# TIGER-AI-Lab/AnyV2V

Measured on NVIDIA H100. Metric: denoising-steps/sec (16f x 512^2 I2VGen-XL, 50 inv + 50 edit PnP sampling), higher is better.
Workload: dtype f16

## Files before the change

anyv2v_b200/csrc/gemm_common.cuh:

```cuda
#pragma once
#include "host_util.cuh"
#include "ptx.cuh"

namespace av2v {

struct GemmP {
  int mode;
  const __half* a;
  const __half* a2;
  const __half* w;
  int M, N, K;
  int lda, lda2, k_split;
  int Hin, Win, chan;
  int Ho, Wo, stride;
  int taps_w, up2, py, px;
  int Cin;
  int F, HW;
  const __half* bias;
  const __half* rowbias;
  int rows_per_rowbias;
  const __half* residual;
  __half* out;
  int ldo;
  int n_slots;
  long long slot_stride;
  int geglu;
  int n_tiles, num_kb;
};

__device__ __forceinline__ float gelu_erf_fast(float g) {
  const float z = fabsf(g) * 0.70710678118654752f;
  float t;
  asm("rcp.approx.ftz.f32 %0, %1;" : "=f"(t) : "f"(fmaf(0.5f, z, 1.0f)));
  float p = fmaf(t, 0.22427836f, -0.69402432f);
  p = fmaf(p, t, 0.45475456f);
  p = fmaf(p, t, 0.26681793f);
  p = fmaf(p, t, 1.01429605f);
  p = fmaf(p, t, -1.26611602f);
  const float e = t * ex2_approx(fmaf(-z, z, p) * 1.4426950408889634f);
  return fmaf(-fabsf(0.5f * g), e, fmaxf(g, 0.0f));
}

__device__ __forceinline__ uint32_t stage_offset(int row, int chunk) {
  return static_cast<uint32_t>(row * 256 + ((chunk ^ (row & 7)) << 4));
}


template <bool kConv>
__device__ __forceinline__ long long out_row_offset(const GemmP& p, int m) {
  if (!kConv || !p.up2) return static_cast<long long>(m) * p.ldo;
  const int j = m % p.Wo, t = m / p.Wo, i = t % p.Ho, n = t / p.Ho;
  return ((static_cast<long long>(n) * 2 * p.Ho + 2 * i + p.py) * (2 * p.Wo) + 2 * j + p.px) * p.ldo;
}

template <bool kConv>
__device__ __forceinline__ void fetch_residual_band(const GemmP& p, int slot, int m0, int n0, int r0, uint32_t tile) {
  const int lane = threadIdx.x & 31, ch = lane & 15;
  const int c = n0 + 8 * ch;
  const __half* src = p.residual + slot * p.slot_stride + c;
#pragma unroll
  for (int i = 0; i < 8; ++i) {
    const int r = r0 + 2 * i + (lane >> 4);
    const bool v = m0 + r < p.M && c < p.N;
    cp_async16(tile + stage_offset(r, ch), v ? src + out_row_offset<kConv>(p, m0 + r) : p.residual, v);
  }
}

template <int kBands>
__device__ __forceinline__ void epilogue_bands(const GemmP& p, const float (&d)[kBands][64], int m0, int n0, int r0,
                                               uint32_t tile) {
  const int fr = r0 + ((threadIdx.x & 31) >> 2);
  const int cq = 2 * (threadIdx.x & 3);
  const __half* rb[kBands][2];
#pragma unroll
  for (int b = 0; b < kBands; ++b)
#pragma unroll
    for (int h = 0; h < 2; ++h) {
      const int m = m0 + fr + 64 * b + 8 * h;
      rb[b][h] = p.rowbias && m < p.M ? p.rowbias + static_cast<long long>(m / p.rows_per_rowbias) * p.N : nullptr;
    }
#pragma unroll
  for (int j = 0; j < 16; ++j) {
    const int c = n0 + 8 * j + cq;
    if (c >= p.N) continue;
    float2 bias = make_float2(0.f, 0.f);
    if (p.bias) bias = __half22float2(*reinterpret_cast<const __half2*>(p.bias + c));
#pragma unroll
    for (int b = 0; b < kBands; ++b)
#pragma unroll
      for (int h = 0; h < 2; ++h) {
        const uint32_t at = tile + stage_offset(fr + 64 * b + 8 * h, j) + 2 * cq;
        float o0 = d[b][4 * j + 2 * h], o1 = d[b][4 * j + 2 * h + 1];
        if (p.bias) {
          o0 += bias.x;
          o1 += bias.y;
        }
        if (rb[b][h]) {
          const float2 t = __half22float2(*reinterpret_cast<const __half2*>(rb[b][h] + c));
          o0 += t.x;
          o1 += t.y;
        }
        if (p.residual) {
          const uint32_t rr = ld_shared_u32(at);
          const float2 r = __half22float2(*reinterpret_cast<const __half2*>(&rr));
          o0 += r.x;
          o1 += r.y;
        }
        st_shared_u32(at, pack_half2(o0, o1));
      }
  }
}

template <bool kConv>
__device__ __forceinline__ void copy_out_band(const GemmP& p, int slot, int m0, int n0, int r0, uint32_t tile) {
  const int lane = threadIdx.x & 31;
  const bool geglu = !kConv && p.geglu;
  const int lg = geglu ? 3 : 4;
  const int col0 = geglu ? n0 / 2 : n0, n_out = geglu ? p.N / 2 : p.N;
  __half* out = p.out + slot * p.slot_stride + col0;
#pragma unroll
  for (int i = 0; i < 8; ++i) {
    const int idx = 32 * i + lane;
    const int r = r0 + (idx >> lg), ch = idx & ((1 << lg) - 1);
    if ((idx >> lg) < 16 && m0 + r < p.M && col0 + 8 * ch < n_out)
      st_global_v4(out + out_row_offset<kConv>(p, m0 + r) + 8 * ch, ld_shared_v4(tile + stage_offset(r, ch)));
  }
}

int gemm_linear_ws(const GemmP& p, int tiles, cudaStream_t stream);
bool conv_ws_box(const GemmP& p, unsigned (&box)[3]);
int gemm_conv_ws(const GemmP& p, const unsigned (&box)[3], int tiles, cudaStream_t stream);

}
```

anyv2v_b200/csrc/gemm_wgmma.cu:

```cuda
#include "gemm_common.cuh"

namespace av2v {
namespace {

constexpr int BM = 128, BN = 128, BK = 64;
constexpr int kStages = 3;
constexpr int kThreads = 256;
constexpr int kTileBytes = BM * BK * 2;
constexpr int kSmemBytes = kStages * 2 * kTileBytes + 1024;

struct ARows {
  long long base[4];
  int y[4], x[4];
};

__device__ __forceinline__ void a_rows_init(const GemmP& p, int m0, int r0, ARows& ar) {
#pragma unroll
  for (int i = 0; i < 4; ++i) {
    const int m = m0 + r0 + 32 * i;
    ar.y[i] = -1 << 20;
    ar.x[i] = 0;
    ar.base[i] = 0;
    if (m >= p.M) continue;
    if (p.mode == AV2V_A_CONV3X3) {
      const int ox = m % p.Wo, t = m / p.Wo, oy = t % p.Ho, n = t / p.Ho;
      const int y0 = p.up2 ? oy - 1 + p.py : oy * p.stride - 1;
      const int x0 = p.up2 ? ox - 1 + p.px : ox * p.stride - 1;
      ar.y[i] = y0;
      ar.x[i] = x0;
      ar.base[i] = (static_cast<long long>(n) * p.Hin + y0) * p.Win + x0;
    } else {
      ar.base[i] = m;
      ar.y[i] = (m % (p.F * p.HW)) / p.HW;
    }
  }
}

__device__ __forceinline__ void load_stage(const GemmP& p, const ARows& ar, int kb, int n0, uint32_t sA, uint32_t sB) {
  const int tid = threadIdx.x;
  const int ch = tid & 7, r0 = tid >> 3;
  const int k0 = kb * BK;
  if (p.mode == AV2V_A_CONV3X3) {
    const int tap = k0 / p.Cin, c = k0 - tap * p.Cin + ch * 8;
    const int ky = tap / p.taps_w, kx = tap - ky * p.taps_w;
    const bool cval = c < p.chan;
#pragma unroll
    for (int i = 0; i < 4; ++i) {
      const int y = ar.y[i] + ky, x = ar.x[i] + kx;
      const bool v = cval && y >= 0 && y < p.Hin && x >= 0 && x < p.Win;
      const __half* src = p.a + (ar.base[i] + static_cast<long long>(ky) * p.Win + kx) * p.chan + c;
      cp_async16(sA + sw128_offset(r0 + 32 * i, ch), v ? src : p.a, v);
    }
  } else {
    const int kt = k0 / p.Cin, c = k0 - kt * p.Cin + ch * 8;
#pragma unroll
    for (int i = 0; i < 4; ++i) {
      const int f = ar.y[i] + kt - 1;
      const bool v = ar.y[i] >= 0 && f >= 0 && f < p.F;
      const __half* src = p.a + (ar.base[i] + static_cast<long long>(kt - 1) * p.HW) * p.Cin + c;
      cp_async16(sA + sw128_offset(r0 + 32 * i, ch), v ? src : p.a, v);
    }
  }
  const bool kval = k0 + ch * 8 < p.K;
#pragma unroll
  for (int i = 0; i < 4; ++i) {
    const int n = n0 + r0 + 32 * i;
    const bool v = kval && n < p.N;
    cp_async16(sB + sw128_offset(r0 + 32 * i, ch), v ? p.w + static_cast<long long>(n) * p.K + k0 + ch * 8 : p.w, v);
  }
}

__global__ void __launch_bounds__(kThreads, 2) gemm_wgmma_kernel(const __grid_constant__ GemmP p) {
  extern __shared__ uint8_t smem_raw[];
  uint8_t* smem = reinterpret_cast<uint8_t*>((reinterpret_cast<uintptr_t>(smem_raw) + 1023) & ~uintptr_t(1023));
  const uint32_t s0 = smem_u32(smem);
  auto sA = [&](int s) { return s0 + static_cast<uint32_t>(s) * 2 * kTileBytes; };
  auto sB = [&](int s) { return s0 + static_cast<uint32_t>(s) * 2 * kTileBytes + kTileBytes; };

  const int n_t = blockIdx.x % p.n_tiles;
  const int m_t = blockIdx.x / p.n_tiles;
  const int m0 = m_t * BM, n0 = n_t * BN;
  const int wg = threadIdx.x >> 7;

  ARows ar;
  a_rows_init(p, m0, threadIdx.x >> 3, ar);

  float d[1][64];
#pragma unroll
  for (int i = 0; i < 64; ++i) d[0][i] = 0.f;

  const int nk = p.num_kb;
#pragma unroll
  for (int s = 0; s < kStages - 2; ++s) {
    if (s < nk) load_stage(p, ar, s, n0, sA(s), sB(s));
    cp_async_commit();
  }
  for (int kb = 0; kb < nk; ++kb) {
    cp_async_wait<kStages - 3>();
    fence_proxy_async_smem();
    __syncthreads();
    {
      const int pf = kb + kStages - 2;
      if (pf < nk) load_stage(p, ar, pf, n0, sA(pf % kStages), sB(pf % kStages));
      cp_async_commit();
    }
    const int s = kb % kStages;
    const uint32_t a_base = sA(s) + wg * 64 * 128;
    const uint32_t b_base = sB(s);
    wgmma_fence();
#pragma unroll
    for (int k = 0; k < BK / 16; ++k)
      wgmma_m64n128_ss(d[0], sw128_desc(a_base + k * 32), sw128_desc(b_base + k * 32), 1);
    wgmma_commit();
    wgmma_wait<1>();
    reg_fence(d[0]);
  }
  const int r0 = 16 * (threadIdx.x >> 5);
  if (p.residual) fetch_residual_band<true>(p, 0, m0, n0, r0, sA(nk % kStages));
  wgmma_wait<0>();
  reg_fence(d[0]);

  const int n_res = p.residual ? p.n_slots : 1;
  if (n_res > 1) {
    __syncthreads();
    for (int s = 1; s < n_res; ++s) fetch_residual_band<true>(p, s, m0, n0, r0, sA((nk + s) % kStages));
  }
  cp_async_commit();
  cp_async_wait<0>();
  __syncwarp();
  for (int s = 0; s < n_res; ++s) epilogue_bands<1>(p, d, m0, n0, r0, sA((nk + s) % kStages));
  __syncwarp();
  for (int s = 0; s < p.n_slots; ++s) copy_out_band<true>(p, s, m0, n0, r0, sA((nk + (p.residual ? s : 0)) % kStages));
}

}
}

using namespace av2v;

extern "C" int av2v_gemm_f16(const av2v_gemm_args* a, av2v_stream_t stream_) {
  cudaStream_t stream = static_cast<cudaStream_t>(stream_);
  AV2V_REQUIRE(a != nullptr, AV2V_EINVAL, "gemm: null args");
  AV2V_REQUIRE(a->a && a->w && a->out, AV2V_EINVAL, "gemm: null a/w/out pointer");
  AV2V_REQUIRE(a->M > 0 && a->N > 0 && a->K > 0, AV2V_EINVAL, "gemm: M,N,K must be positive (%d,%d,%d)", a->M, a->N,
               a->K);
  AV2V_REQUIRE(a->N % 8 == 0 && a->K % 8 == 0, AV2V_EINVAL, "gemm: N and K must be multiples of 8 (%d,%d)", a->N,
               a->K);
  AV2V_REQUIRE((a->geglu || a->ldo >= a->N) && a->ldo % 8 == 0, AV2V_EINVAL,
               "gemm: ldo must be >= N and a multiple of 8");
  AV2V_REQUIRE(a->n_slots >= 1, AV2V_EINVAL, "gemm: n_slots must be >= 1");
  AV2V_REQUIRE(!a->residual || a->n_slots <= kStages, AV2V_ENOSUP, "gemm: at most %d slots with a residual (one staging tile each)", kStages);
  AV2V_REQUIRE(a->n_slots == 1 || a->slot_stride % 8 == 0, AV2V_EALIGN, "gemm: slot_stride must be a multiple of 8");
  AV2V_REQUIRE(aligned16(a->a) && aligned16(a->w) && aligned16(a->out), AV2V_EALIGN,
               "gemm: a/w/out must be 16-byte aligned");
  AV2V_REQUIRE(!a->bias || aligned16(a->bias), AV2V_EALIGN, "gemm: bias must be 16-byte aligned");
  AV2V_REQUIRE(!a->rowbias || (aligned16(a->rowbias) && a->rows_per_rowbias > 0), AV2V_EALIGN,
               "gemm: rowbias must be 16-byte aligned with rows_per_rowbias > 0");
  AV2V_REQUIRE(!a->residual || aligned16(a->residual), AV2V_EALIGN, "gemm: residual must be 16-byte aligned");

  GemmP p{};
  p.mode = a->mode;
  p.a = static_cast<const __half*>(a->a);
  p.w = static_cast<const __half*>(a->w);
  p.M = a->M;
  p.N = a->N;
  p.K = a->K;
  p.bias = static_cast<const __half*>(a->bias);
  p.rowbias = static_cast<const __half*>(a->rowbias);
  p.rows_per_rowbias = a->rows_per_rowbias;
  p.residual = static_cast<const __half*>(a->residual);
  p.out = static_cast<__half*>(a->out);
  p.ldo = a->ldo;
  p.n_slots = a->n_slots;
  p.slot_stride = a->slot_stride;
  p.geglu = a->geglu ? 1 : 0;
  p.stride = 1;
  p.taps_w = 3;
  if (a->geglu) {
    AV2V_REQUIRE(a->mode == AV2V_A_LINEAR, AV2V_EINVAL, "gemm/geglu: LINEAR mode only");
    AV2V_REQUIRE(a->N % 64 == 0, AV2V_EINVAL, "gemm/geglu: N must be a multiple of 64 (got %d)", a->N);
    AV2V_REQUIRE(!a->residual && !a->rowbias && a->n_slots == 1, AV2V_EINVAL, "gemm/geglu: no residual / rowbias / slots");
    AV2V_REQUIRE(a->ldo >= a->N / 2, AV2V_EINVAL, "gemm/geglu: ldo must be >= N/2");
  }
  if (a->mode == AV2V_A_LINEAR) {
    AV2V_REQUIRE((a->a2 != nullptr || a->lda >= a->K) && a->lda % 8 == 0, AV2V_EINVAL, "gemm: lda must be >= K and a multiple of 8");
    p.lda = a->lda;
    p.k_split = a->K;
    if (a->a2 != nullptr) {
      AV2V_REQUIRE(a->k_split > 0 && a->k_split < a->K && a->k_split % BK == 0, AV2V_EINVAL,
                   "gemm: k_split must be a multiple of 64 inside (0, K) (got %d, K = %d)", a->k_split, a->K);
      AV2V_REQUIRE(a->lda >= a->k_split && a->lda2 >= a->K - a->k_split && a->lda2 % 8 == 0 && aligned16(a->a2), AV2V_EINVAL,
                   "gemm: a / a2 row strides must cover their column ranges (multiples of 8), a2 16-byte aligned");
      p.a2 = static_cast<const __half*>(a->a2);
      p.lda2 = a->lda2;
      p.k_split = a->k_split;
    }
    AV2V_REQUIRE(a->n_slots == 1, AV2V_ENOSUP, "gemm/linear: one output slot only (got n_slots = %d)", a->n_slots);
  } else if (a->mode == AV2V_A_CONV3X3) {
    AV2V_REQUIRE(a->NF > 0 && a->H > 0 && a->W > 0 && a->Cin > 0, AV2V_EINVAL, "gemm/conv3x3: bad geometry");
    AV2V_REQUIRE(a->Cin % BK == 0, AV2V_ENOSUP, "gemm/conv3x3: Cin must be a multiple of 64 (got %d)", a->Cin);
    const int up = a->up2_phase;
    AV2V_REQUIRE(up >= 0 && up <= 4, AV2V_EINVAL, "gemm/conv3x3: up2_phase must be 0..4 (got %d)", up);
    AV2V_REQUIRE(a->K == (up ? 4 : 9) * a->Cin, AV2V_EINVAL, "gemm/conv3x3: K must equal 9*Cin (4*Cin for an up2 phase)");
    AV2V_REQUIRE(!up || (a->stride <= 1 && !a->rowbias && !a->residual && a->n_slots == 1), AV2V_EINVAL,
                 "gemm/conv3x3: an up2 phase takes bias only (no stride, rowbias, residual, slots)");
    const int stride = a->stride == 0 ? 1 : a->stride;
    AV2V_REQUIRE(stride == 1 || stride == 2, AV2V_ENOSUP, "gemm/conv3x3: stride must be 1 or 2 (got %d)", a->stride);
    AV2V_REQUIRE(a->H % stride == 0 && a->W % stride == 0, AV2V_ENOSUP, "gemm/conv3x3: H, W must be multiples of the stride");
    const int chan = a->a_channels == 0 ? a->Cin : a->a_channels;
    AV2V_REQUIRE(chan > 0 && chan <= a->Cin && chan % 8 == 0, AV2V_EINVAL, "gemm/conv3x3: a_channels must be a multiple of 8 in (0, Cin]");
    AV2V_REQUIRE(static_cast<long long>(a->NF) * (a->H / stride) * (a->W / stride) == a->M, AV2V_EINVAL,
                 "gemm/conv3x3: M != NF*(H/stride)*(W/stride)");
    p.Hin = a->H;
    p.Win = a->W;
    p.chan = chan;
    p.Ho = a->H / stride;
    p.Wo = a->W / stride;
    p.stride = stride;
    p.Cin = a->Cin;
    if (up) {
      p.up2 = 1;
      p.taps_w = 2;
      p.py = (up - 1) >> 1;
      p.px = (up - 1) & 1;
    }
  } else if (a->mode == AV2V_A_TCONV3) {
    AV2V_REQUIRE(a->B > 0 && a->rows_per_clip > 0 && a->HW > 0 && a->Cin > 0, AV2V_EINVAL, "gemm/tconv3: bad geometry");
    AV2V_REQUIRE(a->Cin % BK == 0, AV2V_ENOSUP, "gemm/tconv3: Cin must be a multiple of 64 (got %d)", a->Cin);
    AV2V_REQUIRE(a->K == 3 * a->Cin, AV2V_EINVAL, "gemm/tconv3: K must equal 3*Cin");
    AV2V_REQUIRE(a->rows_per_clip % a->HW == 0, AV2V_EINVAL, "gemm/tconv3: rows_per_clip must be F*HW");
    AV2V_REQUIRE(static_cast<long long>(a->B) * a->rows_per_clip == a->M, AV2V_EINVAL, "gemm/tconv3: M != B*F*HW");
    p.Cin = a->Cin;
    p.HW = a->HW;
    p.F = a->rows_per_clip / a->HW;
  } else {
    return fail(AV2V_EINVAL, "gemm: unknown A mode %d", a->mode);
  }
  p.num_kb = (a->K + BK - 1) / BK;
  p.n_tiles = (a->N + BN - 1) / BN;
  const long long tiles = static_cast<long long>((a->M + BM - 1) / BM) * p.n_tiles;
  AV2V_REQUIRE(tiles < (1ll << 31), AV2V_ENOSUP, "gemm: too many tiles");
  if (p.mode == AV2V_A_LINEAR) return gemm_linear_ws(p, static_cast<int>(tiles), stream);
  unsigned box[3];
  if (conv_ws_box(p, box)) return gemm_conv_ws(p, box, static_cast<int>(tiles), stream);
  static bool attr_set = false;
  if (!attr_set) {
    AV2V_CHECK_CUDA(cudaFuncSetAttribute(gemm_wgmma_kernel, cudaFuncAttributeMaxDynamicSharedMemorySize, kSmemBytes));
    attr_set = true;
  }
  gemm_wgmma_kernel<<<static_cast<unsigned>(tiles), kThreads, kSmemBytes, stream>>>(p);
  AV2V_CHECK_CUDA(cudaGetLastError());
  return AV2V_OK;
}
```

anyv2v_b200/csrc/gemm_ws.cu:

```cuda
#include "gemm_common.cuh"
#include "ring.cuh"

namespace av2v {
namespace {

constexpr int BM = 128, BN = 128, BK = 64;
constexpr int kStages = 4;
constexpr int kThreads = 384;
constexpr int kTileBytes = BM * BK * 2;
constexpr int kStageBytes = 2 * kTileBytes;
constexpr int kStagingBytes = BM * BN * 2;
constexpr int kSmemBytes = kStages * kStageBytes + 2 * kStagingBytes + 1024;

struct WsP {
  CUtensorMap ta, ta2, tw;
  GemmP g;
  int tiles;
  int ax, ay, x_off, y_off, taps_w;
};

__device__ __forceinline__ void geglu_epilogue(const GemmP& p, float (&d)[2][64], int n0, uint32_t tile) {
  const int cq = 2 * (threadIdx.x & 3);
#pragma unroll
  for (int g = 0; g < 2; ++g) {
#pragma unroll
    for (int jj = 0; jj < 4; ++jj) {
      const int jh = 8 * g + jj, jg = jh + 4;
      const int ch = n0 + 8 * jh + cq, cg = n0 + 8 * jg + cq;
      if (ch >= p.N) continue;
      float2 bh = make_float2(0.f, 0.f), bg = bh;
      if (p.bias) {
        bh = __half22float2(*reinterpret_cast<const __half2*>(p.bias + ch));
        bg = __half22float2(*reinterpret_cast<const __half2*>(p.bias + cg));
      }
#pragma unroll
      for (int half = 0; half < 2; ++half)
#pragma unroll
        for (int h = 0; h < 2; ++h) {
          float h0 = d[half][4 * jh + 2 * h], h1 = d[half][4 * jh + 2 * h + 1];
          float g0 = d[half][4 * jg + 2 * h], g1 = d[half][4 * jg + 2 * h + 1];
          if (p.bias) {
            h0 += bh.x; h1 += bh.y; g0 += bg.x; g1 += bg.y;
          }
          st_shared_u32(tile + stage_offset(64 * half + acc_row(0) + 8 * h, 4 * g + jj) + 2 * cq,
                        pack_half2(h0 * gelu_erf_fast(g0), h1 * gelu_erf_fast(g1)));
        }
    }
  }
}

template <bool kConv>
__global__ void __launch_bounds__(kThreads, 1) gemm_ws_kernel(const __grid_constant__ WsP P) {
  const GemmP& p = P.g;
  extern __shared__ uint8_t smem_raw[];
  __shared__ StageRing<kStages> ring;
  uint8_t* smem = reinterpret_cast<uint8_t*>((reinterpret_cast<uintptr_t>(smem_raw) + 1023) & ~uintptr_t(1023));
  const uint32_t s0 = smem_u32(smem);
  auto sA = [&](int s) { return s0 + static_cast<uint32_t>(s) * kStageBytes; };
  auto sB = [&](int s) { return sA(s) + kTileBytes; };
  const int nk = p.num_kb;
  if (threadIdx.x == 0) {
    ring.init(4);
    fence_mbar_init();
  }
  __syncthreads();

  const int role = __shfl_sync(0xffffffffu, static_cast<int>(threadIdx.x >> 7), 0);
  if (role == 0) {
    setmaxnreg_dec<40>();
    if (threadIdx.x == 0) {
      int g = 0;
      for (int t = blockIdx.x; t < P.tiles; t += gridDim.x) {
        const int m0 = t / p.n_tiles * BM, n0 = t % p.n_tiles * BN;
        int bx = 0, by = 0, bn = 0, c0 = 0, kx = 0;
        if constexpr (kConv) {
          bx = m0 % P.ax + P.x_off;
          by = m0 / P.ax % P.ay + P.y_off;
          bn = m0 / (P.ax * P.ay);
        }
        for (int kb = 0; kb < nk; ++kb, ++g) {
          const int s = ring.stage(g), k0 = kb * BK;
          uint64_t* bar = ring.produce(g, kStageBytes);
          if constexpr (kConv) {
            tma_load_4d(sA(s), &P.ta, bar, c0, bx + kx, by, bn);
            if ((c0 += BK) == p.Cin) {
              c0 = 0;
              if (++kx == P.taps_w) kx = 0, ++by;
            }
          } else if (k0 < p.k_split) tma_load_4d(sA(s), &P.ta, bar, k0, m0, 0, 0);
          else tma_load_4d(sA(s), &P.ta2, bar, k0 - p.k_split, m0, 0, 0);
          tma_load_4d(sB(s), &P.tw, bar, k0, n0, 0, 0);
        }
      }
    }
    return;
  }

  setmaxnreg_inc<232>();
  const int wg = role - 1;
  const uint32_t staging = s0 + kStages * kStageBytes + wg * kStagingBytes;
  turn_open(wg);

  const int r0 = 16 * ((threadIdx.x >> 5) & 3);
  float d[2][64];
  for (int i = wg, t = blockIdx.x + wg * gridDim.x; t < P.tiles; i += 2, t += 2 * gridDim.x) {
    const int m0 = t / p.n_tiles * BM, n0 = t % p.n_tiles * BN;
    if (p.residual)
#pragma unroll
      for (int b = 0; b < 2; ++b) {
        if constexpr (kConv) fetch_residual_band<true>(p, 0, m0, n0, r0 + 64 * b, staging);
        else fetch_residual_band<false>(p, 0, m0, n0, r0 + 64 * b, staging);
      }
    cp_async_commit();
#pragma unroll
    for (int h = 0; h < 2; ++h)
#pragma unroll
      for (int e = 0; e < 64; ++e) d[h][e] = 0.f;
    const int g0 = i * nk;
    turn_take(wg);
    for (int kb = 0; kb < nk; ++kb) {
      const int g = g0 + kb, s = ring.stage(g);
      ring.wait(g);
      wgmma_fence();
#pragma unroll
      for (int k = 0; k < BK / 16; ++k) {
        const uint64_t db = sw128_desc(sB(s) + k * 32);
        wgmma_m64n128_ss(d[0], sw128_desc(sA(s) + k * 32), db, 1);
        wgmma_m64n128_ss(d[1], sw128_desc(sA(s) + 64 * 128 + k * 32), db, 1);
      }
      wgmma_commit();
      wgmma_wait<1>();
      reg_fence(d[0]);
      reg_fence(d[1]);
      if (kb > 0) ring.release(g - 1);
    }
    if (t + gridDim.x < P.tiles) turn_hand_over(wg);
    wgmma_wait<0>();
    reg_fence(d[0]);
    reg_fence(d[1]);
    ring.release(g0 + nk - 1);

    if constexpr (kConv) {
      const int n_res = p.residual ? p.n_slots : 1;
#pragma unroll 1
      for (int sl = 0; sl < n_res; ++sl) {
        if (sl > 0) {
#pragma unroll
          for (int b = 0; b < 2; ++b) fetch_residual_band<true>(p, sl, m0, n0, r0 + 64 * b, staging);
          cp_async_commit();
        }
        cp_async_wait<0>();
        __syncwarp();
        epilogue_bands<2>(p, d, m0, n0, r0, staging);
        __syncwarp();
#pragma unroll 1
        for (int o = p.residual ? sl : 0; o < (p.residual ? sl + 1 : p.n_slots); ++o)
#pragma unroll 1
          for (int b = 0; b < 2; ++b) copy_out_band<true>(p, o, m0, n0, r0 + 64 * b, staging);
        __syncwarp();
      }
    } else {
      cp_async_wait<0>();
      __syncwarp();
      if (p.geglu) geglu_epilogue(p, d, n0, staging);
      else epilogue_bands<2>(p, d, m0, n0, r0, staging);
      __syncwarp();
#pragma unroll
      for (int b = 0; b < 2; ++b) copy_out_band<false>(p, 0, m0, n0, r0 + 64 * b, staging);
      __syncwarp();
    }
  }
}

template <bool kConv>
int launch_ws(const WsP& P, cudaStream_t stream) {
  static bool attr_set = false;
  if (!attr_set) {
    AV2V_CHECK_CUDA(cudaFuncSetAttribute(gemm_ws_kernel<kConv>, cudaFuncAttributeMaxDynamicSharedMemorySize, kSmemBytes));
    attr_set = true;
  }
  const int tiles = P.tiles;
  const int grid = static_cast<int>(tiles < sm_count_cached() ? tiles : sm_count_cached());
  gemm_ws_kernel<kConv><<<grid, kThreads, kSmemBytes, stream>>>(P);
  AV2V_CHECK_CUDA(cudaGetLastError());
  return AV2V_OK;
}

}

int gemm_linear_ws(const GemmP& g, int tiles, cudaStream_t stream) {
  WsP P{};
  P.g = g;
  if (int e = encode_rows_map(&P.ta, g.a, g.k_split, g.M, 1, 1, g.lda, 0, BM)) return e;
  P.ta2 = P.ta;
  if (g.a2 != nullptr)
    if (int e = encode_rows_map(&P.ta2, g.a2, g.K - g.k_split, g.M, 1, 1, g.lda2, 0, BM)) return e;
  if (int e = encode_rows_map(&P.tw, g.w, g.K, g.N, 1, 1, g.K, 0, BN)) return e;
  P.tiles = tiles;
  return launch_ws<false>(P, stream);
}

bool conv_ws_box(const GemmP& p, unsigned (&box)[3]) {
  if (p.mode == AV2V_A_CONV3X3) {
    const int hw = p.Ho * p.Wo;
    if (p.stride != 1 || BM % p.Wo != 0) return false;
    if (hw >= BM) {
      if (hw % BM != 0) return false;
      box[0] = p.Wo, box[1] = BM / p.Wo, box[2] = 1;
    } else {
      if (BM % hw != 0) return false;
      box[0] = p.Wo, box[1] = p.Ho, box[2] = BM / hw;
    }
    return true;
  }
  if (p.mode == AV2V_A_TCONV3) {
    if (p.HW % BM == 0) box[0] = BM, box[1] = 1, box[2] = 1;
    else if (BM % p.HW == 0 && p.F % (BM / p.HW) == 0) box[0] = p.HW, box[1] = BM / p.HW, box[2] = 1;
    else return false;
    return true;
  }
  return false;
}

int gemm_conv_ws(const GemmP& g, const unsigned (&box)[3], int tiles, cudaStream_t stream) {
  WsP P{};
  P.g = g;
  using u64 = unsigned long long;
  const unsigned b4[4] = {64, box[0], box[1], box[2]};
  if (g.mode == AV2V_A_CONV3X3) {
    const u64 row = static_cast<u64>(g.chan) * 2, plane = row * g.Win * g.Hin;
    const u64 dims[4] = {static_cast<u64>(g.chan), static_cast<u64>(g.Win), static_cast<u64>(g.Hin),
                         static_cast<u64>(g.M / (g.Ho * g.Wo))};
    const u64 strides[3] = {row, row * g.Win, plane};
    if (int e = encode_map_4d(&P.ta, g.a, dims, strides, b4)) return e;
    P.ax = g.Wo, P.ay = g.Ho, P.taps_w = g.taps_w;
    P.x_off = g.up2 ? g.px - 1 : -1;
    P.y_off = g.up2 ? g.py - 1 : -1;
  } else {
    const u64 row = static_cast<u64>(g.Cin) * 2;
    const u64 dims[4] = {static_cast<u64>(g.Cin), static_cast<u64>(g.HW), static_cast<u64>(g.F),
                         static_cast<u64>(g.M / (g.F * g.HW))};
    const u64 strides[3] = {row, row * g.HW, row * g.HW * g.F};
    if (int e = encode_map_4d(&P.ta, g.a, dims, strides, b4)) return e;
    P.ax = g.HW, P.ay = g.F, P.taps_w = 1;
    P.x_off = 0;
    P.y_off = -1;
  }
  P.ta2 = P.ta;
  if (int e = encode_rows_map(&P.tw, g.w, g.K, g.N, 1, 1, g.K, 0, BN)) return e;
  P.tiles = tiles;
  return launch_ws<true>(P, stream);
}

}
```

anyv2v_b200/csrc/ptx.cuh:

```cuda
#pragma once
#include <cuda.h>
#include <cuda_fp16.h>
#include <cuda_runtime.h>
#include <cstdint>

namespace av2v {

__device__ __forceinline__ uint32_t smem_u32(const void* p) {
  return static_cast<uint32_t>(__cvta_generic_to_shared(p));
}

__device__ __forceinline__ void mbar_init(uint64_t* bar, uint32_t count) {
  asm volatile("mbarrier.init.shared::cta.b64 [%0], %1;" ::"r"(smem_u32(bar)), "r"(count) : "memory");
}
__device__ __forceinline__ void fence_mbar_init() {
  asm volatile("fence.mbarrier_init.release.cluster;" ::: "memory");
}
__device__ __forceinline__ void fence_proxy_async_smem() {
  asm volatile("fence.proxy.async.shared::cta;" ::: "memory");
}
__device__ __forceinline__ void mbar_arrive_expect_tx(uint64_t* bar, uint32_t bytes) {
  asm volatile("mbarrier.arrive.expect_tx.shared::cta.b64 _, [%0], %1;" ::"r"(smem_u32(bar)), "r"(bytes)
               : "memory");
}
__device__ __forceinline__ void mbar_arrive(uint64_t* bar) {
  asm volatile("mbarrier.arrive.shared::cta.b64 _, [%0];" ::"r"(smem_u32(bar)) : "memory");
}
__device__ __forceinline__ bool mbar_try_wait(uint64_t* bar, uint32_t parity) {
  uint32_t ok;
  asm volatile(
      "{\n"
      ".reg .pred p;\n"
      "mbarrier.try_wait.parity.shared::cta.b64 p, [%1], %2;\n"
      "selp.u32 %0, 1, 0, p;\n"
      "}\n"
      : "=r"(ok)
      : "r"(smem_u32(bar)), "r"(parity)
      : "memory");
  return ok != 0;
}
#ifndef AV2V_WAIT_TIMEOUT_CYCLES
#define AV2V_WAIT_TIMEOUT_CYCLES (4000000000ll)
#endif
template <bool kReport = true>
__device__ __forceinline__ void mbar_wait(uint64_t* bar, uint32_t parity) {
  if (mbar_try_wait(bar, parity)) return;
  const long long t0 = clock64();
  while (!mbar_try_wait(bar, parity)) {
    if (clock64() - t0 > AV2V_WAIT_TIMEOUT_CYCLES) {
      if (kReport)
        printf("av2v: mbarrier wait timeout (block %d,%d thread %d bar %u parity %u)\n", blockIdx.x, blockIdx.y,
               threadIdx.x, smem_u32(bar), parity);
      __trap();
    }
  }
}

__device__ __forceinline__ void tma_load_4d(uint32_t dst, const CUtensorMap* map, uint64_t* bar, int c0, int c1, int c2, int c3) {
  asm volatile(
      "cp.async.bulk.tensor.4d.shared::cluster.global.mbarrier::complete_tx::bytes [%0], [%1, {%2, %3, %4, %5}], [%6];"
      ::"r"(dst), "l"(reinterpret_cast<uint64_t>(map)), "r"(c0), "r"(c1), "r"(c2), "r"(c3), "r"(smem_u32(bar))
      : "memory");
}
__device__ __forceinline__ void named_bar_sync(int id, int threads) {
  asm volatile("bar.sync %0, %1;" ::"r"(id), "r"(threads) : "memory");
}
__device__ __forceinline__ void named_bar_arrive(int id, int threads) {
  asm volatile("bar.arrive %0, %1;" ::"r"(id), "r"(threads) : "memory");
}
template <int R>
__device__ __forceinline__ void setmaxnreg_inc() { asm volatile("setmaxnreg.inc.sync.aligned.u32 %0;" ::"n"(R)); }
template <int R>
__device__ __forceinline__ void setmaxnreg_dec() { asm volatile("setmaxnreg.dec.sync.aligned.u32 %0;" ::"n"(R)); }

__device__ __forceinline__ void cp_async16(uint32_t dst, const void* src, bool valid) {
  asm volatile("cp.async.cg.shared.global [%0], [%1], 16, %2;" ::"r"(dst), "l"(src), "r"(valid ? 16 : 0) : "memory");
}
__device__ __forceinline__ void cp_async_commit() { asm volatile("cp.async.commit_group;" ::: "memory"); }
template <int N>
__device__ __forceinline__ void cp_async_wait() {
  asm volatile("cp.async.wait_group %0;" ::"n"(N) : "memory");
}

__device__ __forceinline__ void st_shared_u32(uint32_t addr, uint32_t v) {
  asm volatile("st.shared.b32 [%0], %1;" ::"r"(addr), "r"(v) : "memory");
}
__device__ __forceinline__ uint32_t ld_shared_u32(uint32_t addr) {
  uint32_t v;
  asm volatile("ld.shared.b32 %0, [%1];" : "=r"(v) : "r"(addr) : "memory");
  return v;
}
__device__ __forceinline__ uint4 ld_shared_v4(uint32_t addr) {
  uint4 v;
  asm volatile("ld.shared.v4.b32 {%0, %1, %2, %3}, [%4];" : "=r"(v.x), "=r"(v.y), "=r"(v.z), "=r"(v.w) : "r"(addr) : "memory");
  return v;
}

__device__ __forceinline__ void st_global_v4(void* p, uint4 v) {
  asm volatile("st.global.v4.b32 [%0], {%1, %2, %3, %4};" ::"l"(p), "r"(v.x), "r"(v.y), "r"(v.z), "r"(v.w) : "memory");
}

__device__ __forceinline__ uint32_t sw128_offset(int row, int chunk) {
  return static_cast<uint32_t>(row * 128 + ((chunk ^ (row & 7)) << 4));
}
__device__ __forceinline__ uint64_t sw128_desc(uint32_t smem_addr) {
  uint64_t d = 0;
  d |= static_cast<uint64_t>((smem_addr & 0x3FFFF) >> 4);
  d |= static_cast<uint64_t>(1) << 16;
  d |= static_cast<uint64_t>(1024 >> 4) << 32;
  d |= static_cast<uint64_t>(1) << 62;
  return d;
}

__device__ __forceinline__ void wgmma_fence() { asm volatile("wgmma.fence.sync.aligned;" ::: "memory"); }
__device__ __forceinline__ void wgmma_commit() { asm volatile("wgmma.commit_group.sync.aligned;" ::: "memory"); }
template <int N>
__device__ __forceinline__ void wgmma_wait() {
  asm volatile("wgmma.wait_group.sync.aligned %0;" ::"n"(N) : "memory");
}
template <int N>
__device__ __forceinline__ void reg_fence(float (&d)[N]) {
#pragma unroll
  for (int i = 0; i < N; ++i) asm volatile("" : "+f"(d[i])::"memory");
}

#define AV2V_WG_D8(i) "+f"(d[i + 0]), "+f"(d[i + 1]), "+f"(d[i + 2]), "+f"(d[i + 3]), "+f"(d[i + 4]), "+f"(d[i + 5]), "+f"(d[i + 6]), "+f"(d[i + 7])

template <int kTransB>
__device__ __forceinline__ void wgmma_m64n64_ss(float (&d)[32], uint64_t da, uint64_t db, int accumulate) {
  asm volatile(
      "{\n.reg .pred p;\nsetp.ne.b32 p, %34, 0;\n"
      "wgmma.mma_async.sync.aligned.m64n64k16.f32.f16.f16 "
      "{%0, %1, %2, %3, %4, %5, %6, %7, %8, %9, %10, %11, %12, %13, %14, %15, "
      "%16, %17, %18, %19, %20, %21, %22, %23, %24, %25, %26, %27, %28, %29, %30, %31}, "
      "%32, %33, p, 1, 1, 0, %35;\n}\n"
      : AV2V_WG_D8(0), AV2V_WG_D8(8), AV2V_WG_D8(16), AV2V_WG_D8(24)
      : "l"(da), "l"(db), "r"(accumulate), "n"(kTransB));
}
template <int kTransB>
__device__ __forceinline__ void wgmma_m64n64_rs(float (&d)[32], const uint32_t (&a)[4], uint64_t db, int accumulate) {
  asm volatile(
      "{\n.reg .pred p;\nsetp.ne.b32 p, %37, 0;\n"
      "wgmma.mma_async.sync.aligned.m64n64k16.f32.f16.f16 "
      "{%0, %1, %2, %3, %4, %5, %6, %7, %8, %9, %10, %11, %12, %13, %14, %15, "
      "%16, %17, %18, %19, %20, %21, %22, %23, %24, %25, %26, %27, %28, %29, %30, %31}, "
      "{%32, %33, %34, %35}, %36, p, 1, 1, %38;\n}\n"
      : AV2V_WG_D8(0), AV2V_WG_D8(8), AV2V_WG_D8(16), AV2V_WG_D8(24)
      : "r"(a[0]), "r"(a[1]), "r"(a[2]), "r"(a[3]), "l"(db), "r"(accumulate), "n"(kTransB));
}
__device__ __forceinline__ void wgmma_m64n128_ss(float (&d)[64], uint64_t da, uint64_t db, int accumulate) {
  asm volatile(
      "{\n.reg .pred p;\nsetp.ne.b32 p, %66, 0;\n"
      "wgmma.mma_async.sync.aligned.m64n128k16.f32.f16.f16 "
      "{%0, %1, %2, %3, %4, %5, %6, %7, %8, %9, %10, %11, %12, %13, %14, %15, "
      "%16, %17, %18, %19, %20, %21, %22, %23, %24, %25, %26, %27, %28, %29, %30, %31, "
      "%32, %33, %34, %35, %36, %37, %38, %39, %40, %41, %42, %43, %44, %45, %46, %47, "
      "%48, %49, %50, %51, %52, %53, %54, %55, %56, %57, %58, %59, %60, %61, %62, %63}, "
      "%64, %65, p, 1, 1, 0, 0;\n}\n"
      : AV2V_WG_D8(0), AV2V_WG_D8(8), AV2V_WG_D8(16), AV2V_WG_D8(24), AV2V_WG_D8(32), AV2V_WG_D8(40), AV2V_WG_D8(48),
        AV2V_WG_D8(56)
      : "l"(da), "l"(db), "r"(accumulate));
}
#undef AV2V_WG_D8

__device__ __forceinline__ int acc_row(int i) { return 16 * ((threadIdx.x & 127) >> 5) + ((threadIdx.x & 31) >> 2) + 8 * ((i >> 1) & 1); }
__device__ __forceinline__ int acc_col(int i) { return 8 * (i >> 2) + 2 * (threadIdx.x & 3) + (i & 1); }

__device__ __forceinline__ uint32_t pack_half2(float lo, float hi) {
  __half2 h = __floats2half2_rn(lo, hi);
  return *reinterpret_cast<uint32_t*>(&h);
}
__device__ __forceinline__ float ex2_approx(float x) {
  float y;
  asm("ex2.approx.ftz.f32 %0, %1;" : "=f"(y) : "f"(x));
  return y;
}

__device__ __forceinline__ float ex2_poly(float x) {
  x = fmaxf(x, -125.0f);
  const float t = x + 12582912.0f;
  const float f = x - (t - 12582912.0f);
  float p = fmaf(f, 0.05517164245247841f, 0.2426111251115799f);
  p = fmaf(p, f, 0.6932609677314758f);
  p = fmaf(p, f, 0.9999280571937561f);
  return __int_as_float(__float_as_int(p) + (__float_as_int(t) << 23));
}

__device__ __forceinline__ float2 ffma2(float2 a, float2 b, float2 c) {
  return make_float2(fmaf(a.x, b.x, c.x), fmaf(a.y, b.y, c.y));
}
__device__ __forceinline__ float2 fadd2(float2 a, float2 b) { return make_float2(__fadd_rn(a.x, b.x), __fadd_rn(a.y, b.y)); }
__device__ __forceinline__ float2 fmul2(float2 a, float2 b) { return make_float2(__fmul_rn(a.x, b.x), __fmul_rn(a.y, b.y)); }

}
```

Measured before the change: 9.490.

## Add 160-wide N tile to warp-specialized GEMM for better wave quantization

Adds a BN=160 variant of the warp-specialized WGMMA GEMM, using m64n160 instructions, a widened staging layout, and residual/copy-out handling for the extra 32 columns. A heuristic chooses 160 when N is divisible by 160 and the padded per-SM work is no larger than with 128-wide tiles. This targets wave-quantization waste for channel counts like 320, 640 and 1280. The cost is more accumulator registers and more shared memory per stage, and GEGLU layers stay on the 128 path.

```diff
diff --git a/anyv2v_b200/csrc/gemm_common.cuh b/anyv2v_b200/csrc/gemm_common.cuh
--- a/anyv2v_b200/csrc/gemm_common.cuh
+++ b/anyv2v_b200/csrc/gemm_common.cuh
@@ -41,8 +41,11 @@
   return fmaf(-fabsf(0.5f * g), e, fmaxf(g, 0.0f));
 }
 
+template <int kBN = 128>
 __device__ __forceinline__ uint32_t stage_offset(int row, int chunk) {
-  return static_cast<uint32_t>(row * 256 + ((chunk ^ (row & 7)) << 4));
+  static_assert(kBN == 128 || kBN == 160, "staging tiles are 128 or 160 columns wide");
+  if (kBN == 128 || chunk < 16) return static_cast<uint32_t>(row * 256 + ((chunk ^ (row & 7)) << 4));
+  return static_cast<uint32_t>(128 * 256 + row * 64 + (((chunk - 16) ^ ((row >> 1) & 3)) << 4));
 }
 
 
@@ -53,7 +56,7 @@
   return ((static_cast<long long>(n) * 2 * p.Ho + 2 * i + p.py) * (2 * p.Wo) + 2 * j + p.px) * p.ldo;
 }
 
-template <bool kConv>
+template <bool kConv, int kBN = 128>
 __device__ __forceinline__ void fetch_residual_band(const GemmP& p, int slot, int m0, int n0, int r0, uint32_t tile) {
   const int lane = threadIdx.x & 31, ch = lane & 15;
   const int c = n0 + 8 * ch;
@@ -62,13 +65,24 @@
   for (int i = 0; i < 8; ++i) {
     const int r = r0 + 2 * i + (lane >> 4);
     const bool v = m0 + r < p.M && c < p.N;
-    cp_async16(tile + stage_offset(r, ch), v ? src + out_row_offset<kConv>(p, m0 + r) : p.residual, v);
+    cp_async16(tile + stage_offset<kBN>(r, ch), v ? src + out_row_offset<kConv>(p, m0 + r) : p.residual, v);
+  }
+  if constexpr (kBN == 160) {
+    const int ct = 16 + (lane & 3), c1 = n0 + 8 * ct;
+#pragma unroll
+    for (int i = 0; i < 2; ++i) {
+      const int r = r0 + 8 * i + (lane >> 2);
+      const bool v = m0 + r < p.M && c1 < p.N;
+      cp_async16(tile + stage_offset<kBN>(r, ct),
+                 v ? p.residual + slot * p.slot_stride + c1 + out_row_offset<kConv>(p, m0 + r) : p.residual, v);
+    }
   }
 }
 
-template <int kBands>
-__device__ __forceinline__ void epilogue_bands(const GemmP& p, const float (&d)[kBands][64], int m0, int n0, int r0,
+template <int kBands, int kAcc>
+__device__ __forceinline__ void epilogue_bands(const GemmP& p, const float (&d)[kBands][kAcc], int m0, int n0, int r0,
                                                uint32_t tile) {
+  constexpr int kBN = 2 * kAcc;
   const int fr = r0 + ((threadIdx.x & 31) >> 2);
   const int cq = 2 * (threadIdx.x & 3);
   const __half* rb[kBands][2];
@@ -80,7 +94,7 @@
       rb[b][h] = p.rowbias && m < p.M ? p.rowbias + static_cast<long long>(m / p.rows_per_rowbias) * p.N : nullptr;
     }
 #pragma unroll
-  for (int j = 0; j < 16; ++j) {
+  for (int j = 0; j < kBN / 8; ++j) {
     const int c = n0 + 8 * j + cq;
     if (c >= p.N) continue;
     float2 bias = make_float2(0.f, 0.f);
@@ -89,7 +103,7 @@
     for (int b = 0; b < kBands; ++b)
 #pragma unroll
       for (int h = 0; h < 2; ++h) {
-        const uint32_t at = tile + stage_offset(fr + 64 * b + 8 * h, j) + 2 * cq;
+        const uint32_t at = tile + stage_offset<kBN>(fr + 64 * b + 8 * h, j) + 2 * cq;
         float o0 = d[b][4 * j + 2 * h], o1 = d[b][4 * j + 2 * h + 1];
         if (p.bias) {
           o0 += bias.x;
@@ -111,10 +125,10 @@
   }
 }
 
-template <bool kConv>
+template <bool kConv, int kBN = 128>
 __device__ __forceinline__ void copy_out_band(const GemmP& p, int slot, int m0, int n0, int r0, uint32_t tile) {
   const int lane = threadIdx.x & 31;
-  const bool geglu = !kConv && p.geglu;
+  const bool geglu = kBN == 128 && !kConv && p.geglu;
   const int lg = geglu ? 3 : 4;
   const int col0 = geglu ? n0 / 2 : n0, n_out = geglu ? p.N / 2 : p.N;
   __half* out = p.out + slot * p.slot_stride + col0;
@@ -123,10 +137,20 @@
     const int idx = 32 * i + lane;
     const int r = r0 + (idx >> lg), ch = idx & ((1 << lg) - 1);
     if ((idx >> lg) < 16 && m0 + r < p.M && col0 + 8 * ch < n_out)
-      st_global_v4(out + out_row_offset<kConv>(p, m0 + r) + 8 * ch, ld_shared_v4(tile + stage_offset(r, ch)));
+      st_global_v4(out + out_row_offset<kConv>(p, m0 + r) + 8 * ch, ld_shared_v4(tile + stage_offset<kBN>(r, ch)));
+  }
+  if constexpr (kBN == 160) {
+    const int ct = 16 + (lane & 3);
+#pragma unroll
+    for (int i = 0; i < 2; ++i) {
+      const int r = r0 + 8 * i + (lane >> 2);
+      if (m0 + r < p.M && n0 + 8 * ct < p.N)
+        st_global_v4(out + out_row_offset<kConv>(p, m0 + r) + 8 * ct, ld_shared_v4(tile + stage_offset<kBN>(r, ct)));
+    }
   }
 }
 
+int ws_tile_n(const GemmP& p);
 int gemm_linear_ws(const GemmP& p, int tiles, cudaStream_t stream);
 bool conv_ws_box(const GemmP& p, unsigned (&box)[3]);
 int gemm_conv_ws(const GemmP& p, const unsigned (&box)[3], int tiles, cudaStream_t stream);
diff --git a/anyv2v_b200/csrc/gemm_wgmma.cu b/anyv2v_b200/csrc/gemm_wgmma.cu
--- a/anyv2v_b200/csrc/gemm_wgmma.cu
+++ b/anyv2v_b200/csrc/gemm_wgmma.cu
@@ -237,12 +237,14 @@
     return fail(AV2V_EINVAL, "gemm: unknown A mode %d", a->mode);
   }
   p.num_kb = (a->K + BK - 1) / BK;
-  p.n_tiles = (a->N + BN - 1) / BN;
+  unsigned box[3];
+  const bool ws = p.mode == AV2V_A_LINEAR || conv_ws_box(p, box);
+  const int bn = ws ? ws_tile_n(p) : BN;
+  p.n_tiles = (a->N + bn - 1) / bn;
   const long long tiles = static_cast<long long>((a->M + BM - 1) / BM) * p.n_tiles;
   AV2V_REQUIRE(tiles < (1ll << 31), AV2V_ENOSUP, "gemm: too many tiles");
   if (p.mode == AV2V_A_LINEAR) return gemm_linear_ws(p, static_cast<int>(tiles), stream);
-  unsigned box[3];
-  if (conv_ws_box(p, box)) return gemm_conv_ws(p, box, static_cast<int>(tiles), stream);
+  if (ws) return gemm_conv_ws(p, box, static_cast<int>(tiles), stream);
   static bool attr_set = false;
   if (!attr_set) {
     AV2V_CHECK_CUDA(cudaFuncSetAttribute(gemm_wgmma_kernel, cudaFuncAttributeMaxDynamicSharedMemorySize, kSmemBytes));
diff --git a/anyv2v_b200/csrc/gemm_ws.cu b/anyv2v_b200/csrc/gemm_ws.cu
--- a/anyv2v_b200/csrc/gemm_ws.cu
+++ b/anyv2v_b200/csrc/gemm_ws.cu
@@ -4,13 +4,14 @@
 namespace av2v {
 namespace {
 
-constexpr int BM = 128, BN = 128, BK = 64;
+constexpr int BM = 128, BK = 64;
 constexpr int kStages = 4;
 constexpr int kThreads = 384;
 constexpr int kTileBytes = BM * BK * 2;
-constexpr int kStageBytes = 2 * kTileBytes;
-constexpr int kStagingBytes = BM * BN * 2;
-constexpr int kSmemBytes = kStages * kStageBytes + 2 * kStagingBytes + 1024;
+template <int kBN> constexpr int kStageBytes = kTileBytes + kBN * BK * 2;
+template <int kBN> constexpr int kStagingBytes = BM * kBN * 2;
+template <int kBN> constexpr int kSmemBytes = kStages * kStageBytes<kBN> + 2 * kStagingBytes<kBN> + 1024;
+static_assert(kSmemBytes<160> <= 227 * 1024, "the 160-wide ring and staging tiles must fit an SM's shared memory");
 
 struct WsP {
   CUtensorMap ta, ta2, tw;
@@ -49,14 +50,15 @@
   }
 }
 
-template <bool kConv>
+template <bool kConv, int kBN>
 __global__ void __launch_bounds__(kThreads, 1) gemm_ws_kernel(const __grid_constant__ WsP P) {
+  constexpr int kStage = kStageBytes<kBN>, kStaging = kStagingBytes<kBN>;
   const GemmP& p = P.g;
   extern __shared__ uint8_t smem_raw[];
   __shared__ StageRing<kStages> ring;
   uint8_t* smem = reinterpret_cast<uint8_t*>((reinterpret_cast<uintptr_t>(smem_raw) + 1023) & ~uintptr_t(1023));
   const uint32_t s0 = smem_u32(smem);
-  auto sA = [&](int s) { return s0 + static_cast<uint32_t>(s) * kStageBytes; };
+  auto sA = [&](int s) { return s0 + static_cast<uint32_t>(s) * kStage; };
   auto sB = [&](int s) { return sA(s) + kTileBytes; };
   const int nk = p.num_kb;
   if (threadIdx.x == 0) {
@@ -71,7 +73,7 @@
     if (threadIdx.x == 0) {
       int g = 0;
       for (int t = blockIdx.x; t < P.tiles; t += gridDim.x) {
-        const int m0 = t / p.n_tiles * BM, n0 = t % p.n_tiles * BN;
+        const int m0 = t / p.n_tiles * BM, n0 = t % p.n_tiles * kBN;
         int bx = 0, by = 0, bn = 0, c0 = 0, kx = 0;
         if constexpr (kConv) {
           bx = m0 % P.ax + P.x_off;
@@ -80,7 +82,7 @@
         }
         for (int kb = 0; kb < nk; ++kb, ++g) {
           const int s = ring.stage(g), k0 = kb * BK;
-          uint64_t* bar = ring.produce(g, kStageBytes);
+          uint64_t* bar = ring.produce(g, kStage);
           if constexpr (kConv) {
             tma_load_4d(sA(s), &P.ta, bar, c0, bx + kx, by, bn);
             if ((c0 += BK) == p.Cin) {
@@ -98,24 +100,24 @@
 
   setmaxnreg_inc<232>();
   const int wg = role - 1;
-  const uint32_t staging = s0 + kStages * kStageBytes + wg * kStagingBytes;
+  const uint32_t staging = s0 + kStages * kStage + wg * kStaging;
   turn_open(wg);
 
   const int r0 = 16 * ((threadIdx.x >> 5) & 3);
-  float d[2][64];
+  float d[2][kBN / 2];
   for (int i = wg, t = blockIdx.x + wg * gridDim.x; t < P.tiles; i += 2, t += 2 * gridDim.x) {
-    const int m0 = t / p.n_tiles * BM, n0 = t % p.n_tiles * BN;
+    const int m0 = t / p.n_tiles * BM, n0 = t % p.n_tiles * kBN;
     if (p.residual)
 #pragma unroll
       for (int b = 0; b < 2; ++b) {
-        if constexpr (kConv) fetch_residual_band<true>(p, 0, m0, n0, r0 + 64 * b, staging);
-        else fetch_residual_band<false>(p, 0, m0, n0, r0 + 64 * b, staging);
+        if constexpr (kConv) fetch_residual_band<true, kBN>(p, 0, m0, n0, r0 + 64 * b, staging);
+        else fetch_residual_band<false, kBN>(p, 0, m0, n0, r0 + 64 * b, staging);
       }
     cp_async_commit();
 #pragma unroll
     for (int h = 0; h < 2; ++h)
 #pragma unroll
-      for (int e = 0; e < 64; ++e) d[h][e] = 0.f;
+      for (int e = 0; e < kBN / 2; ++e) d[h][e] = 0.f;
     const int g0 = i * nk;
     turn_take(wg);
     for (int kb = 0; kb < nk; ++kb) {
@@ -125,8 +127,13 @@
 #pragma unroll
       for (int k = 0; k < BK / 16; ++k) {
         const uint64_t db = sw128_desc(sB(s) + k * 32);
-        wgmma_m64n128_ss(d[0], sw128_desc(sA(s) + k * 32), db, 1);
-        wgmma_m64n128_ss(d[1], sw128_desc(sA(s) + 64 * 128 + k * 32), db, 1);
+        if constexpr (kBN == 128) {
+          wgmma_m64n128_ss(d[0], sw128_desc(sA(s) + k * 32), db, 1);
+          wgmma_m64n128_ss(d[1], sw128_desc(sA(s) + 64 * 128 + k * 32), db, 1);
+        } else {
+          wgmma_m64n160_ss(d[0], sw128_desc(sA(s) + k * 32), db, 1);
+          wgmma_m64n160_ss(d[1], sw128_desc(sA(s) + 64 * 128 + k * 32), db, 1);
+        }
       }
       wgmma_commit();
       wgmma_wait<1>();
@@ -146,7 +153,7 @@
       for (int sl = 0; sl < n_res; ++sl) {
         if (sl > 0) {
 #pragma unroll
-          for (int b = 0; b < 2; ++b) fetch_residual_band<true>(p, sl, m0, n0, r0 + 64 * b, staging);
+          for (int b = 0; b < 2; ++b) fetch_residual_band<true, kBN>(p, sl, m0, n0, r0 + 64 * b, staging);
           cp_async_commit();
         }
         cp_async_wait<0>();
@@ -156,36 +163,50 @@
 #pragma unroll 1
         for (int o = p.residual ? sl : 0; o < (p.residual ? sl + 1 : p.n_slots); ++o)
 #pragma unroll 1
-          for (int b = 0; b < 2; ++b) copy_out_band<true>(p, o, m0, n0, r0 + 64 * b, staging);
+          for (int b = 0; b < 2; ++b) copy_out_band<true, kBN>(p, o, m0, n0, r0 + 64 * b, staging);
         __syncwarp();
       }
     } else {
       cp_async_wait<0>();
       __syncwarp();
-      if (p.geglu) geglu_epilogue(p, d, n0, staging);
-      else epilogue_bands<2>(p, d, m0, n0, r0, staging);
+      if constexpr (kBN == 128) {
+        if (p.geglu) geglu_epilogue(p, d, n0, staging);
+        else epilogue_bands<2>(p, d, m0, n0, r0, staging);
+      } else {
+        epilogue_bands<2>(p, d, m0, n0, r0, staging);
+      }
       __syncwarp();
 #pragma unroll
-      for (int b = 0; b < 2; ++b) copy_out_band<false>(p, 0, m0, n0, r0 + 64 * b, staging);
+      for (int b = 0; b < 2; ++b) copy_out_band<false, kBN>(p, 0, m0, n0, r0 + 64 * b, staging);
       __syncwarp();
     }
   }
 }
 
-template <bool kConv>
-int launch_ws(const WsP& P, cudaStream_t stream) {
+template <bool kConv, int kBN>
+int launch_ws(WsP P, cudaStream_t stream) {
+  const GemmP& g = P.g;
+  if (int e = encode_rows_map(&P.tw, g.w, g.K, g.N, 1, 1, g.K, 0, kBN)) return e;
   static bool attr_set = false;
   if (!attr_set) {
-    AV2V_CHECK_CUDA(cudaFuncSetAttribute(gemm_ws_kernel<kConv>, cudaFuncAttributeMaxDynamicSharedMemorySize, kSmemBytes));
+    AV2V_CHECK_CUDA(cudaFuncSetAttribute(gemm_ws_kernel<kConv, kBN>, cudaFuncAttributeMaxDynamicSharedMemorySize,
+                                         kSmemBytes<kBN>));
     attr_set = true;
   }
   const int tiles = P.tiles;
   const int grid = static_cast<int>(tiles < sm_count_cached() ? tiles : sm_count_cached());
-  gemm_ws_kernel<kConv><<<grid, kThreads, kSmemBytes, stream>>>(P);
+  gemm_ws_kernel<kConv, kBN><<<grid, kThreads, kSmemBytes<kBN>, stream>>>(P);
   AV2V_CHECK_CUDA(cudaGetLastError());
   return AV2V_OK;
 }
 
+}
+
+int ws_tile_n(const GemmP& p) {
+  if (p.geglu || p.N % 160 != 0) return 128;
+  const long long mt = (p.M + BM - 1) / BM, sms = sm_count_cached();
+  const long long t128 = (mt * ((p.N + 127) / 128) + sms - 1) / sms * 128, t160 = (mt * (p.N / 160) + sms - 1) / sms * 160;
+  return t160 <= t128 ? 160 : 128;
 }
 
 int gemm_linear_ws(const GemmP& g, int tiles, cudaStream_t stream) {
@@ -195,9 +216,8 @@
   P.ta2 = P.ta;
   if (g.a2 != nullptr)
     if (int e = encode_rows_map(&P.ta2, g.a2, g.K - g.k_split, g.M, 1, 1, g.lda2, 0, BM)) return e;
-  if (int e = encode_rows_map(&P.tw, g.w, g.K, g.N, 1, 1, g.K, 0, BN)) return e;
   P.tiles = tiles;
-  return launch_ws<false>(P, stream);
+  return ws_tile_n(g) == 160 ? launch_ws<false, 160>(P, stream) : launch_ws<false, 128>(P, stream);
 }
 
 bool conv_ws_box(const GemmP& p, unsigned (&box)[3]) {
@@ -247,9 +267,8 @@
     P.y_off = -1;
   }
   P.ta2 = P.ta;
-  if (int e = encode_rows_map(&P.tw, g.w, g.K, g.N, 1, 1, g.K, 0, BN)) return e;
   P.tiles = tiles;
-  return launch_ws<true>(P, stream);
-}
-
-}
+  return ws_tile_n(g) == 160 ? launch_ws<true, 160>(P, stream) : launch_ws<true, 128>(P, stream);
+}
+
+}
diff --git a/anyv2v_b200/csrc/ptx.cuh b/anyv2v_b200/csrc/ptx.cuh
--- a/anyv2v_b200/csrc/ptx.cuh
+++ b/anyv2v_b200/csrc/ptx.cuh
@@ -161,6 +161,20 @@
         AV2V_WG_D8(56)
       : "l"(da), "l"(db), "r"(accumulate));
 }
+__device__ __forceinline__ void wgmma_m64n160_ss(float (&d)[80], uint64_t da, uint64_t db, int accumulate) {
+  asm volatile(
+      "{\n.reg .pred p;\nsetp.ne.b32 p, %82, 0;\n"
+      "wgmma.mma_async.sync.aligned.m64n160k16.f32.f16.f16 "
+      "{%0, %1, %2, %3, %4, %5, %6, %7, %8, %9, %10, %11, %12, %13, %14, %15, "
+      "%16, %17, %18, %19, %20, %21, %22, %23, %24, %25, %26, %27, %28, %29, %30, %31, "
+      "%32, %33, %34, %35, %36, %37, %38, %39, %40, %41, %42, %43, %44, %45, %46, %47, "
+      "%48, %49, %50, %51, %52, %53, %54, %55, %56, %57, %58, %59, %60, %61, %62, %63, "
+      "%64, %65, %66, %67, %68, %69, %70, %71, %72, %73, %74, %75, %76, %77, %78, %79}, "
+      "%80, %81, p, 1, 1, 0, 0;\n}\n"
+      : AV2V_WG_D8(0), AV2V_WG_D8(8), AV2V_WG_D8(16), AV2V_WG_D8(24), AV2V_WG_D8(32), AV2V_WG_D8(40), AV2V_WG_D8(48),
+        AV2V_WG_D8(56), AV2V_WG_D8(64), AV2V_WG_D8(72)
+      : "l"(da), "l"(db), "r"(accumulate));
+}
 #undef AV2V_WG_D8
 
 __device__ __forceinline__ int acc_row(int i) { return 16 * ((threadIdx.x & 127) >> 5) + ((threadIdx.x & 31) >> 2) + 8 * ((i >> 1) & 1); }
```

After: 10.12, median of 6. 6.6% higher.
